# savage-hacker14/audio-to-sheet-music

Hardware: AMD Instinct MI355X
Metric: 6s-segments/sec (each separated into 4 stems; encode once, decode 4x) (higher is better)
Workload: dtype bf16; 1 GPU; BASELINE configs[2]: B=64 x 6 s segments x 4 prompts per GPU; global_batch=64, seq_len=264600, prompts=4, parallelism=segment-sharded dp1, launch=hipGraph replay of one athd_forward_prompts per step (1 graph(s) per rank), pipelines=1, decode_items=256

## Files before the change

audio-to-sheet-music_amd/csrc/fdec_lr.hip:

```cpp
#include <algorithm>
#include <cstdlib>

#include "common.h"
#include "kernels.h"
#include "prof.h"

namespace athd {

namespace {

typedef float f2 __attribute__((ext_vector_type(2)));
typedef __bf16 bf2_t __attribute__((ext_vector_type(2)));

ATHD_DEV f2 splat(float v) { return (f2){v, v}; }
ATHD_DEV f2 pfma(f2 a, f2 b, f2 c) { return __builtin_elementwise_fma(a, b, c); }

template <typename T>
ATHD_DEV f2 ld2(const T* p) {
    if constexpr (sizeof(T) == 2) {
        const uint32_t q = *reinterpret_cast<const uint32_t*>(p);
        return (f2){__uint_as_float(q << 16), __uint_as_float(q & 0xFFFF0000u)};
    } else {
        return *reinterpret_cast<const f2*>(p);
    }
}

template <bool FAST>
ATHD_DEV f2 gelu2(f2 x) {
    if constexpr (!FAST) {
        return (f2){gelu_erf(x.x), gelu_erf(x.y)};
    } else {
        return (f2){gelu_fast(x.x), gelu_fast(x.y)};
    }
}

ATHD_DEV f2 gelu2_pk(f2 x) {
    const f2 u = x * pfma(splat(0.044715f * 1.5957691216057308f), x * x, splat(1.5957691216057308f));
    const f2 t = u * splat(-1.4426950408889634f);
    const f2 den = (f2){__builtin_amdgcn_exp2f(t.x), __builtin_amdgcn_exp2f(t.y)} + splat(1.0f);
    return x * (f2){__builtin_amdgcn_rcpf(den.x), __builtin_amdgcn_rcpf(den.y)};
}

template <typename ZT, int NT>
ATHD_DEV void load_rows(const ZT* base, int64_t rowpitch, int Co, int i0, int i1, float scale, f2 (&r0)[NT],
                        f2 (&dr)[NT]);

template <int NT>
ATHD_DEV constexpr int tap_of(int t) { return NT == 8 ? t : (t == 0 ? 0 : t == 1 ? 3 : t == 2 ? 4 : 7); }

template <typename ZT, int NT>
ATHD_DEV void load_rows(const ZT* base, int64_t rowpitch, int Co, int i0, int i1, float scale, f2 (&r0)[NT],
                        f2 (&dr)[NT]) {
    f2 a[NT], b[NT];
#pragma unroll
    for (int t = 0; t < NT; ++t) a[t] = ld2(base + (int64_t)i0 * rowpitch + tap_of<NT>(t) * Co);
#pragma unroll
    for (int t = 0; t < NT; ++t) b[t] = ld2(base + (int64_t)i1 * rowpitch + tap_of<NT>(t) * Co);
#pragma unroll
    for (int t = 0; t < NT; ++t) {
        r0[t] = a[t] * splat(scale);
        dr[t] = (b[t] - a[t]) * splat(scale);
    }
}

struct LrThread {
    int item, seg, w, c;
    bool active;
};

ATHD_DEV LrThread lr_thread(const LowRankDesc& d) {
    LrThread t;
    const int cg = d.Co / 2;
    const int q = blockIdx.x * 256 + threadIdx.x;
    t.active = q < d.W * cg;
    t.w = t.active ? q / cg : 0;
    t.c = t.active ? (q % cg) * 2 : 0;
    t.item = blockIdx.y;
    t.seg = t.item / d.P;
    return t;
}

}

typedef uint32_t u32x4_t __attribute__((ext_vector_type(4)));
typedef __attribute__((address_space(4))) const u32x4_t c_u32x4;
ATHD_DEV LrStep lr_step(const LrStep* steps, int v) {
    static_assert(sizeof(LrStep) == 32, "LrStep layout");
    const c_u32x4* p = (const c_u32x4*)steps + 2 * __builtin_amdgcn_readfirstlane(v);
    const u32x4_t a = p[0], b = p[1];
    LrStep e;
    e.lz = __uint_as_float(a.x);
    e.lk = __uint_as_float(a.y);
    e.lj = __uint_as_float(a.z);
    e.zk = a.w;
    e.jj = b.x;
    e.flags = b.y;
    return e;
}

__global__ __launch_bounds__(256) void fdec_lr_steps_kernel(LrStep* steps, int Hd, int Hs, int Hk, int H_skip) {
    for (int v = threadIdx.x; v <= Hd; v += blockDim.x) {
        LrStep e = {};
        int z0 = -1, z1 = -1, k0 = -1, k1 = -1, j0 = -1, j1 = -1, pz0 = -2, pz1 = -2, pk0 = -2, pk1 = -2, pj0 = -2,
            pj1 = -2;
        if (v < Hd) {
            const LinIdx a = lin_index(v, Hs, Hd), k = lin_index(v, Hk, Hd);
            z0 = a.i0; z1 = a.i1; k0 = k.i0; k1 = k.i1;
            e.lz = a.l1;
            e.lk = k.l1;
        }
        if (v >= 1) {
            const LinIdx j = lin_index(v - 1, H_skip, Hd);
            j0 = j.i0; j1 = j.i1;
            e.lj = j.l1;
            if (v - 1 < Hd) {
                const LinIdx pa = lin_index(v - 1, Hs, Hd), pk = lin_index(v - 1, Hk, Hd);
                pz0 = pa.i0; pz1 = pa.i1; pk0 = pk.i0; pk1 = pk.i1;
            }
            if (v >= 2) {
                const LinIdx pj = lin_index(v - 2, H_skip, Hd);
// ... 55 lines not shown
                    const f2 y1 = T[3] + prev[3];
                    a1 += y0 + y1;
                    a2 = pfma(y0, y0, pfma(y1, y1, a2));
                }
#pragma unroll
                for (int t = 0; t < 4; ++t) prev[t] = T[4 + t];
            }
            s1 += (double)a1.x + (double)a1.y;
            s2 += (double)a2.x + (double)a2.y;
        }
    }
    s1 = wave_sum_d(s1);
    s2 = wave_sum_d(s2);
    __shared__ double sh[2][4];
    const int wv = threadIdx.x >> 6;
    if ((threadIdx.x & 63) == 0) { sh[0][wv] = s1; sh[1][wv] = s2; }
    __syncthreads();
    if (threadIdx.x == 0) {
        atomicAdd(&d.stats[2 * th.item], sh[0][0] + sh[0][1] + sh[0][2] + sh[0][3]);
        atomicAdd(&d.stats[2 * th.item + 1], sh[1][0] + sh[1][1] + sh[1][2] + sh[1][3]);
    }
}

ATHD_DEV f2 bf2u(uint32_t q) { return (f2){__uint_as_float(q << 16), __uint_as_float(q & 0xFFFF0000u)}; }

__global__ __launch_bounds__(256) void fdec_lr_stats3_kernel(const LowRankDesc d) {
    const LrThread th = lr_thread(d);
    const int N8 = 8 * d.Co;
    const int64_t rp = (int64_t)d.W * N8;
    const bf16_t* zb = (const bf16_t*)d.Z + (int64_t)th.item * d.Hs * rp + (int64_t)th.w * N8 + th.c;
    const bf16_t* sb = (const bf16_t*)d.Zs + (int64_t)th.seg * d.Hk * rp + (int64_t)th.w * N8 + th.c;
    const f2 bias = ld2(d.bias + th.c);
    f2 zhi[8], zdr[8], shi[8], sdr[8], base[8];
    uint32_t zpf[8], spf[8];
    double s1 = 0.0, s2 = 0.0;
    auto ldrow = [&](const bf16_t* p, int row, uint32_t (&r)[8]) {
#pragma unroll
        for (int t = 0; t < 8; ++t) r[t] = *reinterpret_cast<const uint32_t*>(p + (int64_t)row * rp + t * d.Co);
    };
    if (th.active) {
        const LrStep s0 = lr_step(d.steps, 0);
        int zr = (s0.zk >> 8) & 0xFF, kr = s0.zk >> 24;
        {
            uint32_t za[8], ka[8];
            ldrow(zb, s0.zk & 0xFF, za);
            ldrow(zb, zr, zpf);
            ldrow(sb, (s0.zk >> 16) & 0xFF, ka);
            ldrow(sb, kr, spf);
// ... 68 lines not shown
            a1 = f2{};
            a2 = f2{};
        }
        a1 += pv[0] + pv[1];
        a2 = pfma(pv[0], pv[0], pfma(pv[1], pv[1], a2));
        s1 += (double)a1.x + (double)a1.y;
        s2 += (double)a2.x + (double)a2.y;
    }
    s1 = wave_sum_d(s1);
    s2 = wave_sum_d(s2);
    __shared__ double sh[2][4];
    const int wv = threadIdx.x >> 6;
    if ((threadIdx.x & 63) == 0) { sh[0][wv] = s1; sh[1][wv] = s2; }
    __syncthreads();
    if (threadIdx.x == 0) {
        atomicAdd(&d.stats[2 * th.item], sh[0][0] + sh[0][1] + sh[0][2] + sh[0][3]);
        atomicAdd(&d.stats[2 * th.item + 1], sh[1][0] + sh[1][1] + sh[1][2] + sh[1][3]);
    }
}

__global__ __launch_bounds__(256) void fdec_lr_merge3_kernel(const LowRankDesc d) {
    const LrThread th = lr_thread(d);
    if (!th.active) return;
    constexpr int NT = 4;
    const int N8 = 8 * d.Co, NZ = d.z_taps * d.Co;
    const int64_t rp = (int64_t)d.W * N8, rpz = (int64_t)d.W * NZ;
    const bool z4 = d.z_taps == 4;
    const bf16_t* zb = (const bf16_t*)d.Z + (int64_t)th.item * d.Hs * rpz + (int64_t)th.w * NZ +
                       (z4 ? (th.c >> 4) * 64 + (th.c & 15) : th.c);
    const bf16_t* sb = (const bf16_t*)d.Zs + (int64_t)th.seg * d.Hk * rp + (int64_t)th.w * N8 + th.c;
    float mean, rstd;
    gn_params(d.stats, th.item, 4LL * d.Hd * d.W * d.Co, mean, rstd);
    const f2 bias = ld2(d.bias + th.c);
    const f2 gsc = ld2(d.gn_w + th.c) * splat(rstd);
    const f2 gb = ld2(d.gn_b + th.c) - splat(mean) * gsc;
    const int64_t kp = (int64_t)d.W * d.C_skip;
    const bf16_t* kbp = (const bf16_t*)d.skip + (int64_t)th.seg * d.H_skip * kp + (int64_t)th.w * d.C_skip + th.c;
    bf2_t* op = (bf2_t*)((bf16_t*)d.out + (int64_t)th.item * d.Hd * d.W * d.Co + (int64_t)th.w * d.Co + th.c);
    const int64_t ostep = (int64_t)d.W * d.Co / 2;

    auto ldrow = [&](const bf16_t* p, int row, uint32_t (&r)[NT], bool compact) {
#pragma unroll
        for (int t = 0; t < NT; ++t)
            r[t] = *reinterpret_cast<const uint32_t*>(p + (int64_t)row * (compact ? rpz : rp) +
                                                      (compact ? t * 16 : tap_of<NT>(t) * d.Co));
    };
    f2 zhi[NT], zdr[NT], shi[NT], sdr[NT], base[NT];
    uint32_t zpf[NT], spf[NT];
    const LrStep s0 = lr_step(d.steps, 0);
    int zr = (s0.zk >> 8) & 0xFF, kr = s0.zk >> 24;
    {
        uint32_t za[NT], ka[NT];
        ldrow(zb, s0.zk & 0xFF, za, z4);
        ldrow(zb, zr, zpf, z4);
        ldrow(sb, (s0.zk >> 16) & 0xFF, ka, false);
        ldrow(sb, kr, spf, false);
#pragma unroll
        for (int t = 0; t < NT; ++t) {
            const f2 a = bf2u(za[t]), b = bf2u(zpf[t]);
            const f2 ka2 = bf2u(ka[t]) * splat(0.1f), kb2 = bf2u(spf[t]) * splat(0.1f);
            zhi[t] = b;
            zdr[t] = b - a;
            shi[t] = kb2;
            sdr[t] = kb2 - ka2;
            base[t] = a + ka2 + ((t == 1 || t == 2) ? bias : f2{});
        }
    }
    ldrow(zb, min(zr + 1, d.Hs - 1), zpf, z4);
    ldrow(sb, min(kr + 1, d.Hk - 1), spf, false);
    const LrStep s1e = lr_step(d.steps, 1);
    int jr = (int)(s1e.jj >> 16);
    f2 khi, kdr;
    uint32_t jpf;
    {
        const f2 a = bf2u(*reinterpret_cast<const uint32_t*>(kbp + (int64_t)(s1e.jj & 0xFFFF) * kp)) * splat(0.1f);
        khi = bf2u(*reinterpret_cast<const uint32_t*>(kbp + (int64_t)jr * kp)) * splat(0.1f);
        kdr = khi - a;
    }
    jpf = *reinterpret_cast<const uint32_t*>(kbp + (int64_t)min(jr + 1, d.H_skip - 1) * kp);
    f2 kbase = khi - kdr;

    auto tstep = [&](const LrStep& st, f2 (&T)[NT]) {
        if (st.flags & 1u) {
#pragma unroll
            for (int t = 0; t < NT; ++t) {
                const f2 nb = bf2u(zpf[t]);
                base[t] += zdr[t];
                zdr[t] = nb - zhi[t];
                zhi[t] = nb;
            }
            zr = min(zr + 1, d.Hs - 1);
            ldrow(zb, min(zr + 1, d.Hs - 1), zpf, z4);
        }
        if (st.flags & 2u) {
#pragma unroll
            for (int t = 0; t < NT; ++t) {
                const f2 nb = bf2u(spf[t]) * splat(0.1f);
                base[t] += sdr[t];
                sdr[t] = nb - shi[t];
                shi[t] = nb;
            }
            kr = min(kr + 1, d.Hk - 1);
            ldrow(sb, min(kr + 1, d.Hk - 1), spf, false);
        }
#pragma unroll
        for (int t = 0; t < NT; ++t) T[t] = pfma(splat(st.lz), zdr[t], pfma(splat(st.lk), sdr[t], base[t]));
    };
    auto emit = [&](const LrStep& st, f2 y1, f2 y2, int dd) {
        if (dd >= 1 && (st.flags & 4u)) {
            const f2 nb = bf2u(jpf) * splat(0.1f);
            kbase += kdr;
            kdr = nb - khi;
            khi = nb;
            jr = min(jr + 1, d.H_skip - 1);
            jpf = *reinterpret_cast<const uint32_t*>(kbp + (int64_t)min(jr + 1, d.H_skip - 1) * kp);
        }
        const f2 gs = gelu_fast_wsum_pk(splat(0.5f), pfma(y1, gsc, gb), splat(0.5f), pfma(y2, gsc, gb));
        const f2 o = gs + pfma(splat(st.lj), kdr, kbase);
        op[(int64_t)dd * ostep] = __builtin_convertvector(o, bf2_t);
    };
    f2 cur3, cur4, cur7, prev7 = {};
    {
        f2 T[NT];
#pragma unroll
        for (int t = 0; t < NT; ++t) T[t] = pfma(splat(s0.lz), zdr[t], pfma(splat(s0.lk), sdr[t], base[t]));
        cur3 = T[1];
        cur4 = T[2];
        cur7 = T[3];
    }
    LrStep nx = s1e;
    for (int v = 1; v < d.Hd; ++v) {
        const LrStep st = nx;
        nx = lr_step(d.steps, v + 1);
        f2 T[NT];
        tstep(st, T);
        emit(st, cur3 + prev7, cur4 + T[0], v - 1);
        prev7 = cur7;
        cur3 = T[1];
        cur4 = T[2];
        cur7 = T[3];
    }
    emit(nx, cur3 + prev7, cur4, d.Hd - 1);
}

template <typename ZT, bool FAST>
__global__ __launch_bounds__(256) void fdec_lr_merge2_kernel(const LowRankDesc d) {
    const LrThread th = lr_thread(d);
    if (!th.active) return;
    const int N8 = 8 * d.Co;
    const int64_t rp = (int64_t)d.W * N8;
    const ZT* zb = (const ZT*)d.Z + (int64_t)th.item * d.Hs * rp + (int64_t)th.w * N8 + th.c;
    const ZT* sb = (const ZT*)d.Zs + (int64_t)th.seg * d.Hk * rp + (int64_t)th.w * N8 + th.c;
    float mean, rstd;
    gn_params(d.stats, th.item, 4LL * d.Hd * d.W * d.Co, mean, rstd);
    const f2 bias = ld2(d.bias + th.c);
    const f2 gsc = ld2(d.gn_w + th.c) * splat(rstd);
    const f2 gb = ld2(d.gn_b + th.c);
    const int64_t kp = (int64_t)d.W * d.C_skip;
    const int64_t kb = (int64_t)th.seg * d.H_skip * kp + (int64_t)th.w * d.C_skip + th.c;
    f2 ka = {}, kd = {};
    const int64_t ob = (int64_t)th.item * d.Hd * d.W * d.Co + (int64_t)th.w * d.Co + th.c;
    const int64_t op = (int64_t)d.W * d.Co;

    f2 zr0[4], zdr[4], sr0[4], sdr[4];
    f2 base[4];
// ... 126 lines not shown
```

audio-to-sheet-music_amd/csrc/forward.h:

```cpp
#pragma once
#include <hip/hip_runtime.h>

#include <algorithm>
#include <cstdio>
#include <cstdlib>
#include <string>
#include <vector>

#include "../../include/athd.h"
#include "attn.h"
#include "ctx.h"
#include "gemm.h"
#include "kernels.h"
#include "prof.h"

namespace athd_fwd {

struct Dims {
    int64_t B = 0, T = 0;
    int P = 1, Tspec = 0;
    int F[5] = {2048, 512, 128, 32, 8};
    int64_t L[5] = {0, 0, 0, 0, 0};
    int64_t Nf = 0, Nt = 0, Nmax = 0;
    int64_t Bc = 0, chunks = 0;
// ... 19 lines not shown
    float *avec, *tc0, *tc2;
    float *Yb, *x_cond, *xt_cond;
    void* Hm;
    float* Ybt;
    void* Hmt;
    float *G, *D, *FO;
    float* FO2 = nullptr;
    float* ola_part;
    LrStep* lrsteps;
    float* gram;
    double* gramq;
    void *S, *Z, *Zs;
    float* skw[2] = {nullptr, nullptr};
};

inline void* eoff(void* p, int64_t n, int ea) { return (char*)p + n * ea; }

struct Switches {
    static bool env(const char* name, bool dflt) {
        const char* e = std::getenv(name);
        return dflt ? !(e && *e == '0') : (e && *e && *e != '0');
    }
    bool serial = env("ATHD_SERIAL", false), sk = env("ATHD_SK", true), rowln = env("ATHD_ROWLN", true),
         fdec1_fused = env("ATHD_FDEC1_FUSED", true), fenc_row = env("ATHD_FENC_ROW", true);
};

struct Status {
    int err = 0;
    std::string what;
    void check(int rc, const char* w) { if (rc != 0 && err == 0) { err = rc; what = w; } }
};

enum Branch { MAIN = 0, TIME = 1 };
struct StreamPlan {
    hipStream_t main, time;
    hipEvent_t ev_f, ev_t;
    bool serial;
    Status* st;

    StreamPlan(athd_ctx* c, hipStream_t caller, bool serial_, Status* st_)
        : main(caller), time(serial_ ? caller : c->s_time), ev_f(c->ev_f), ev_t(c->ev_t), serial(serial_), st(st_) {
        if (!c->s_time || !c->ev_f || !c->ev_t) st->check((int)hipErrorInvalidResourceHandle, "second stream");
    }
    void record(hipEvent_t ev, hipStream_t s) { st->check((int)hipEventRecord(ev, s), "event record"); }
    void wait(hipStream_t s, hipEvent_t ev) { st->check((int)hipStreamWaitEvent(s, ev, 0), "event wait"); }
    void fork() { record(ev_f, main); wait(time, ev_f); }
    void join() { record(ev_t, time); wait(main, ev_t); }
// ... 74 lines not shown
```

audio-to-sheet-music_amd/csrc/forward_dec.cpp:

```cpp
#include "forward.h"

namespace athd_fwd {
namespace {

void conv_t(Run& r, const DecW& w, const void* A, int a_bf16, int nb, int H_in, int W, void* out, int out_bf16,
            double* st, int keep, const char* stage) {
    KStage kst(stage);
    if (w.ct4w && a_bf16 && out_bf16 && convt4_supported(w.cin, w.cout, nb, H_in, W)) {
        ConvT4Desc q;
        q.x = (const uint16_t*)A; q.w = w.ct4w; q.bias = w.ct4b; q.out = (uint16_t*)out; q.stats = st;
        q.nb = nb; q.H = H_in; q.W = W; q.keep = keep < 0 ? 0 : 1;
        r.check(convt4_launch(q, r.s), "convt4");
        return;
    }
    auto residues = [&](const GemmW& gw, int ntaps, int in_off) {
        GemmDesc g = conv_h(gw, A, a_bf16, nb, H_in, W, w.cin, ntaps, 1, in_off, 1, H_in);
        out_to(g, out, out_bf16, w.cout, (keep < 0 ? 4 : 2) * H_in);
        g.o_stride = keep < 0 ? 4 : 2;
        g.stats = st; g.col_split = w.cout;
        return g;
    };
    if (w.quad.w) {
        GemmDesc g = residues(w.quad, 3, -1);
        if (w.cin % 32 == 0) g.k_blk = w.cin;
// ... 58 lines not shown
    else gn_gelu_launch(b.G, NI, 32 * Ts * 192, 192, st, c->fdec[0].gnw, c->fdec[0].gnb, r.s, false);
    KStage kst1("fdec1");
    const DecW& w1 = c->fdec[1];
    GemmDesc gz = conv1(w1.taps, r.actbf ? b.S : (const void*)b.G, ab, NI, 32, Ts, w1.cin);
    out_to(gz, b.Z, ab, w1.taps.N, 32);
    LowRankDesc lr;
    lr.steps = b.lrsteps;
    lr.Z = b.Z; lr.Zs = b.Zs; lr.z_bf16 = ab; lr.Hs = 32; lr.Hk = 8; lr.Hd = (int)Ts; lr.W = (int)Ts;
    lr.Co = w1.cout; lr.P = P; lr.NI = NI; lr.bias = w1.bias; lr.stats = r.stats(NI);
    lr.gn_w = w1.gnw; lr.gn_b = w1.gnb; lr.fast_gelu = ab;
    lr.skip = sv[2]; lr.skip_bf16 = ab; lr.H_skip = 32; lr.C_skip = 192;
    lr.out = b.D; lr.out_bf16 = ab;
    lr.S = gz.A; lr.Wt = w1.taps.w; lr.w_ld = w1.taps.Kp; lr.Ci = w1.cin;
    const bool gram = r.sw.fdec1_fused && b.gram && fdec1_gram_supported(lr);
    if (gram) { lr.z_taps = 4; lr.z4 = b.Z; }
    else r.gemm(gz, "fdec1.z");
    GemmDesc gs = conv1(w1.taps, sv[3], ab, Bc, 8, Ts, w1.cin);
    gs.a_ld = 384;
    out_to(gs, b.Zs, ab, w1.taps.N, 8);
    r.gemm(gs, "fdec1.zs");
    r.check(fdec_lr_steps_launch(b.lrsteps, (int)Ts, 32, 8, 32, r.s), "fdec_lr_steps");
    if (gram) r.check(fdec1_gram_launch(lr, b.gram, b.gramq, r.s), "fdec1_gram");
    else r.check(fdec_lr_stats_launch(lr, r.s), "fdec_lr_stats");
    r.check(fdec_lr_merge_launch(lr, r.s), "fdec_lr_merge");
    const DecW& w = c->fdec[2];
    double* sti = r.stats(NI);
    conv_t(r, w, b.D, ab, NI, (int)Ts, (int)Ts, b.G, ab, sti, 1, "fdec2");
    KStage kst3("fdec3");
    DecLastDesc dl;
    dl.g = b.G; dl.g_bf16 = ab; dl.stats = sti; dl.gn_count = 4 * Ts * Ts * w.cout; dl.gn_w = w.gnw; dl.gn_b = w.gnb;
    dl.fast_gelu = ab; dl.skip2 = sv[1]; dl.skip2_bf16 = ab; dl.H_skip2 = 128; dl.C_skip2 = 96;
    dl.H = (int)Ts; dl.W = (int)Ts;
    last_level(dl, c->flast, eoff(b.sk4, s0 * 512 * Ts * 4, ea), 512);
    dl.out = FO;
    r.check(fdec_tail_launch(dl, r.s), "fdec_tail");
}

float* Chunk::time_decoder() const {
    const void* svt[4] = {eoff(b.saved_t[0], s0 * d.L[1] * 48, b.ea), eoff(b.saved_t[1], s0 * d.L[2] * 96, b.ea),
                          eoff(b.saved_t[2], s0 * d.L[3] * 192, b.ea), eoff(b.saved_t[3], s0 * d.L[4] * 384, b.ea)};
    const void* const sk4t = eoff(b.sk4t, s0 * d.L[1] * 4, b.ea);
    const void* A = b.xt_cond;
    int64_t Lin = d.Nt;
    static const char* const kT[3] = {"tdec0", "tdec1", "tdec2"};
    for (int i = 0; i < 3; ++i) {
        const DecW& w = c->tdec[i];
        double* st = r.stats(NI);
        conv_t(r, w, A, ab, NI, (int)Lin, 1, b.Gt, ab, st, -1, kT[i]);
        KStage kst(kT[i]);
        const int64_t target = d.L[3 - i];
// ... 61 lines not shown
```

audio-to-sheet-music_amd/csrc/kernels.h:

```cpp
#pragma once
#include <hip/hip_runtime.h>
#include <stdint.h>

#include "../../include/athd.h"
#include "gemm.h"

namespace athd {

struct PadPlan {
    int64_t L;
    int64_t left;
    int64_t ext_left;
    int64_t Lx;
};
inline PadPlan stft_pad_plan(int64_t T, int64_t Tspec) {
    const int64_t pl = 1536, pr = 1536 + Tspec * 1024 - T, maxpad = pl > pr ? pl : pr;
    const int64_t extra = T <= maxpad ? maxpad - T + 1 : 0, epr = pr < extra ? pr : extra, epl = extra - epr;
    PadPlan pp;
    pp.L = T; pp.left = pl - epl; pp.ext_left = epl; pp.Lx = T + epl + epr;
    return pp;
}

void tconv0_launch(const float* wav, int nb, int64_t T, int64_t Lo, const float* w, const float* bias,
                   const float* tnorm, void* out, int out_bf16, hipStream_t s);
// ... 105 lines not shown
    float* out = nullptr;
    const void* g = nullptr; int g_bf16 = 0; int Hg = 0;
    const double* stats = nullptr; int64_t gn_count = 0; const float* gn_w = nullptr; const float* gn_b = nullptr;
    int fast_gelu = 0;
    const void* skip2 = nullptr; int skip2_bf16 = 0; int H_skip2 = 0; int C_skip2 = 0;
};
int fdec_last_launch(const DecLastDesc& d, hipStream_t s);
int tdec_last_launch(const DecLastDesc& d, hipStream_t s);
int fdec_tail_launch(const DecLastDesc& d, hipStream_t s);
bool tdec_tail_supported(const DecLastDesc& d);
int tdec_tail_launch(const DecLastDesc& d, hipStream_t s);
struct ConvT4Desc {
    const uint16_t* x = nullptr;
    const uint16_t* w = nullptr;
    const float* bias = nullptr;
    uint16_t* out = nullptr;
    double* stats = nullptr;
    int nb = 0, H = 0, W = 1, keep = 0;
    uint32_t M = 0;
    FastDivU fd_w, fd_h, fd_hw;
};
bool convt4_supported(int cin, int cout, int64_t nb, int64_t H, int64_t W);
int convt4_launch(const ConvT4Desc& d, hipStream_t s);
inline bool dconv_narrow(int C) { return C == 48 || C == 96; }
inline bool dconv_bf16(int mode) { return mode == 1; }
struct DconvPlan {
    bool ok;
    bool valu;
    bool conv3_mfma;
    enum Norm { MOM, BF16, F32 } norm;
    bool apply_mfma;
    bool rewrite;
};
DconvPlan dconv_plan(int mode, int C, int64_t nb, int64_t L, bool rewrite_fusable);
struct DconvDesc {
    void* x = nullptr; int x_bf16 = 0;
    float* h = nullptr;
    uint16_t* hb = nullptr;
    double *st_h = nullptr, *st_y = nullptr;
    int64_t M = 0, L = 0; int C = 0, dil = 1;
    const float *w3f = nullptr, *w1f = nullptr;
    bool fast = false;
    const uint16_t *w3 = nullptr, *w1 = nullptr;
    int w3_kp = 0, w1_kp = 0;
    const float *b3 = nullptr, *g1w = nullptr, *g1b = nullptr, *scale = nullptr;
    const float *b1 = nullptr, *g2w = nullptr, *g2b = nullptr;
// ... 105 lines not shown
```

audio-to-sheet-music_amd/csrc/ktest.cpp:

```cpp
#include <hip/hip_runtime.h>
#include <stdint.h>
#include <string.h>

#include "attn.h"
#include "ctx.h"
#include "forward.h"
#include "gemm.h"
#include "kernels.h"
#include "pack.h"
#include "text_tower.h"

namespace athd {
int dec_merge_run();
int dec_merge_maxp();
int dec_last_const(int which);
int fdec1_gram_wb();
int fdec1_gram_blocks();
}

using namespace athd;

extern "C" {

struct KtGemm {
// ... 257 lines not shown
    d.C_skip = (int)k->C_skip; d.P = (int)k->P; d.out = k->out; d.out_bf16 = (int)k->out_bf16; d.H_out = (int)k->H_out;
    d.W = (int)k->W; d.NI = (int)k->NI; d.proj_w = (const float*)k->proj_w; d.proj_b = (const float*)k->proj_b;
    d.fast_gelu = (int)k->fast_gelu;
    return dec_merge_launch(d, (hipStream_t)stream);
}
static LowRankDesc to_lr(const KtLowRank* k) {
    LowRankDesc d;
    d.steps = (const LrStep*)k->steps; d.Z = k->Z; d.Zs = k->Zs; d.z_bf16 = (int)k->z_bf16; d.z_taps = (int)k->z_taps;
    d.Hs = (int)k->Hs; d.Hk = (int)k->Hk; d.Hd = (int)k->Hd; d.W = (int)k->W; d.Co = (int)k->Co; d.P = (int)k->P;
    d.NI = (int)k->NI; d.bias = (const float*)k->bias; d.stats = (double*)k->stats; d.gn_w = (const float*)k->gn_w;
    d.gn_b = (const float*)k->gn_b; d.fast_gelu = (int)k->fast_gelu; d.skip = k->skip; d.skip_bf16 = (int)k->skip_bf16;
    d.H_skip = (int)k->H_skip; d.C_skip = (int)k->C_skip; d.out = k->out; d.out_bf16 = (int)k->out_bf16;
    d.S = k->S; d.Wt = k->Wt; d.w_ld = (int)k->w_ld; d.Ci = (int)k->Ci; d.z4 = k->z4;
    return d;
}
int kt_fdec_lr_stats(const KtLowRank* k, void* stream) { return fdec_lr_stats_launch(to_lr(k), (hipStream_t)stream); }
int kt_fdec_lr_merge(const KtLowRank* k, void* stream) { return fdec_lr_merge_launch(to_lr(k), (hipStream_t)stream); }
int kt_fdec1_gram(const KtLowRank* k, void* stream) {
    return fdec1_gram_launch(to_lr(k), (float*)k->gram, (double*)k->gq, (hipStream_t)stream);
}
int kt_fdec1_gram_supported(const KtLowRank* k) { return fdec1_gram_supported(to_lr(k)); }
int kt_fdec_lr_steps(void* steps, int64_t Hd, int64_t Hs, int64_t Hk, int64_t H_skip, void* stream) {
    return fdec_lr_steps_launch((LrStep*)steps, (int)Hd, (int)Hs, (int)Hk, (int)H_skip, (hipStream_t)stream);
}
int64_t kt_fdec1_gram_floats(int64_t NI, int64_t W) { return fdec1_gram_floats(NI, (int)W); }
int64_t kt_fdec1_gram_q_doubles() { return fdec1_gram_q_doubles(); }
static DecLastDesc to_dl(const KtDecLast* k) {
    DecLastDesc d;
    d.in = k->in; d.in_bf16 = (int)k->in_bf16; d.NI = (int)k->NI; d.P = (int)k->P; d.H = (int)k->H; d.W = (int)k->W;
    d.T = k->T; d.fold = (const float*)k->fold; d.skip = k->skip; d.skip_bf16 = (int)k->skip_bf16;
    d.H_skip = (int)k->H_skip; d.C_skip = (int)k->C_skip; d.out = (float*)k->out; d.g = k->g; d.g_bf16 = (int)k->g_bf16;
    d.Hg = (int)k->Hg; d.stats = (const double*)k->stats; d.gn_count = k->gn_count; d.gn_w = (const float*)k->gn_w;
    d.gn_b = (const float*)k->gn_b; d.fast_gelu = (int)k->fast_gelu; d.skip2 = k->skip2; d.skip2_bf16 = (int)k->skip2_bf16;
    d.H_skip2 = (int)k->H_skip2; d.C_skip2 = (int)k->C_skip2;
    return d;
}
int kt_fdec_last(const KtDecLast* k, void* stream) { return fdec_last_launch(to_dl(k), (hipStream_t)stream); }
int kt_tdec_last(const KtDecLast* k, void* stream) { return tdec_last_launch(to_dl(k), (hipStream_t)stream); }
int kt_fdec_tail(const KtDecLast* k, void* stream) { return fdec_tail_launch(to_dl(k), (hipStream_t)stream); }
int kt_tdec_tail(const KtDecLast* k, void* stream) { return tdec_tail_launch(to_dl(k), (hipStream_t)stream); }
int kt_tdec_tail_supported(const KtDecLast* k) { return tdec_tail_supported(to_dl(k)); }
int64_t kt_fl_dc() { return dec_last_const(0); }
int64_t kt_ft_dc() { return dec_last_const(1); }
int64_t kt_tl_in() { return dec_last_const(2); }
int64_t kt_tt_rows() { return dec_last_const(3); }
int64_t kt_dm_run() { return dec_merge_run(); }
// ... 176 lines not shown
```

Baseline: 1853 segments/s.

## Fuse low-rank merge with fdec2 transposed conv via LDS ring producer/consumer kernel

```diff
diff --git a/audio-to-sheet-music_amd/csrc/fdec12.hip b/audio-to-sheet-music_amd/csrc/fdec12.hip
--- /dev/null
+++ b/audio-to-sheet-music_amd/csrc/fdec12.hip
@@ -0,0 +1,198 @@
+#include <algorithm>
+
+#include "common.h"
+#include "fdec_lr_merge3.h"
+#include "gemm.h"
+#include "gemm_tile.h"
+#include "kernels.h"
+#include "prof.h"
+
+namespace athd {
+
+namespace {
+
+constexpr int CT_CI = 96, CT_CO = 48;
+constexpr int CT_KP = 2 * CT_CI;
+constexpr int CT_WROW = CT_KP * 2;
+constexpr int F12_R = FDEC12_R, F12_SLOTS = 2 * F12_R;
+constexpr int F12_ROWB = FDEC12_WB * CT_CI * 2;
+constexpr int F12_NP = 12, F12_NC = 4;
+constexpr int F12_OSB = FDEC12_WB * CT_CO * 2;
+static_assert((F12_SLOTS & (F12_SLOTS - 1)) == 0, "ring slots: a power of two");
+static_assert(F12_NP * 64 == FDEC12_WB * (CT_CI / 2), "one producer thread per (column, channel pair)");
+
+ATHD_DEV int ring_chunk(int w, int ch) { return (ch & 12) | ((ch ^ (0 - (w >> 2))) & 3); }
+
+}
+
+__global__ __launch_bounds__(1024) void fdec12_kernel(const LowRankDesc d, const ConvT4Desc q, const Fdec12Plan plan) {
+    __shared__ __attribute__((aligned(16))) char wl[4 * CT_CO * CT_WROW];
+    __shared__ __attribute__((aligned(16))) char ring[F12_SLOTS * F12_ROWB];
+    __shared__ __attribute__((aligned(16))) char ostg[2][F12_OSB];
+    __shared__ double ssum[2][F12_NC][2];
+    if (fdec12_task(plan, (int)blockIdx.x, 0) < 0) return;
+    for (int c = threadIdx.x; c < 4 * CT_CO * 24; c += 1024) {
+        const int n = c / 24, ch = c - 24 * (c / 24);
+        const uint4 v = reinterpret_cast<const uint4*>(q.w)[c];
+        *reinterpret_cast<uint4*>(wl + n * CT_WROW + ((ch ^ (n & 7)) * 16)) = v;
+    }
+    __syncthreads();
+
+    const int lane = threadIdx.x & 63;
+    const int wave = __builtin_amdgcn_readfirstlane(threadIdx.x >> 6);
+    const int Hd = d.Hd, W = d.W;
+    const int phases = plan.phases;
+
+    if (wave < F12_NP) {
+        const int wl_ = threadIdx.x / (CT_CI / 2), c = (threadIdx.x % (CT_CI / 2)) * 2;
+        char* const slot0 = ring + wl_ * (CT_CI * 2) + ring_chunk(wl_, c >> 3) * 16 + (c & 7) * 2;
+        for (int k = 0;; ++k) {
+            const int t = fdec12_task(plan, (int)blockIdx.x, k);
+            if (t < 0) break;
+            const int wblk = t / d.NI, item = t - wblk * d.NI;
+            const int w = min(FDEC12_WB * wblk + wl_, W - 1);
+            lr_merge3_rows(d, item, item / d.P, w, c, [&](int dd, bf2_t v) {
+                *reinterpret_cast<bf2_t*>(slot0 + (dd & (F12_SLOTS - 1)) * F12_ROWB) = v;
+                if (((dd + 1) & (F12_R - 1)) == 0) __syncthreads();
+            });
+            for (int ph = Hd / F12_R; ph < phases; ++ph) __syncthreads();
+        }
+        return;
+    }
+
+    const int rho = wave - F12_NP;
+    const int fr = lane & 15, g = lane >> 4;
+    const bool stored = rho == 1 || rho == 2;
+    float4 b4[3];
+#pragma unroll
+    for (int jj = 0; jj < 3; ++jj) b4[jj] = *reinterpret_cast<const float4*>(q.bias + 16 * jj + 4 * g);
+    const int f7 = fr & 7;
+    const uint32_t wrho = (uint32_t)((96 * (rho >> 1) + 16 * 3 * (rho & 1)) * CT_WROW);
+    uint32_t wbe = wrho + (uint32_t)(fr * CT_WROW + (4 * (f7 >> 2) + (g ^ (f7 & 3))) * 16);
+    uint32_t wbo = wrho + (uint32_t)(fr * CT_WROW + (4 * (1 - (f7 >> 2)) + (g ^ (f7 & 3))) * 16);
+    auto wfrag = [&](int jj, int s) -> bf16v8 {
+        const uint32_t a = ((s & 1) ? wbo : wbe) + (uint32_t)(16 * jj * CT_WROW + 128 * (s >> 1));
+        return *reinterpret_cast<const bf16v8*>(wl + a);
+    };
+    const uint32_t roff = (uint32_t)(fr * (CT_CI * 2) + ring_chunk(fr, g) * 16);
+    const f32x4_t z4 = {0.f, 0.f, 0.f, 0.f};
+    f32x4_t acc[3];
+    bf16v8 wf[3][3];
+    auto wload = [&](int gi) {
+        __builtin_amdgcn_sched_barrier(0);
+#pragma unroll
+        for (int jj = 0; jj < 3; ++jj) wf[gi % 3][jj] = wfrag(jj, gi);
+        __builtin_amdgcn_sched_barrier(0);
+    };
+    auto mma = [&](int h, const bf16v8 (&F)[3]) {
+#pragma unroll
+        for (int s = 0; s < 3; ++s) {
+#pragma unroll
+            for (int jj = 0; jj < 3; ++jj)
+                acc[jj] = __builtin_amdgcn_mfma_f32_16x16x32_bf16(wf[s][jj], F[s], (h == 0 && s == 0) ? z4 : acc[jj], 0, 0, 0);
+            wload((3 * h + s + 3) % 6);
+        }
+    };
+    wload(0);
+    wload(1);
+    wload(2);
+    const bf16v8 zf = __builtin_bit_cast(bf16v8, make_uint4(0u, 0u, 0u, 0u));
+    char* const stage = ostg[stored ? rho - 1 : 0];
+
+    for (int k = 0;; ++k) {
+        const int t = fdec12_task(plan, (int)blockIdx.x, k);
+        if (t < 0) break;
+        const int wblk = t / d.NI, item = t - wblk * d.NI;
+        const bool cok = FDEC12_WB * wblk + fr < W;
+        char* const oitem = reinterpret_cast<char*>(q.out) + (int64_t)item * Hd * 2 * W * (CT_CO * 2);
+        const int64_t orowB = (int64_t)W * (CT_CO * 2);
+        const int ocol0 = FDEC12_WB * wblk * (CT_CO * 2);
+        const int ovalid = min(FDEC12_WB, W - FDEC12_WB * wblk) * (CT_CO * 2);
+        double r1 = 0.0, r2 = 0.0;
+        bf16v8 lo[3] = {zf, zf, zf}, up[3];
+        __syncthreads();
+        for (int ph = 1; ph < phases; ++ph) {
+            const int rend = min(ph * F12_R, Hd + 1);
+#pragma unroll 1
+            for (int r = (ph - 1) * F12_R; r < rend; ++r) {
+                if (r < Hd) {
+                    const char* const rp = ring + (r & (F12_SLOTS - 1)) * F12_ROWB + roff;
+#pragma unroll
+                    for (int s3 = 0; s3 < 3; ++s3) up[s3] = *reinterpret_cast<const bf16v8*>(rp + 64 * s3);
+                } else {
+#pragma unroll
+                    for (int s3 = 0; s3 < 3; ++s3) up[s3] = zf;
+                }
+                const int u = rho < 2 ? r : r - 1;
+                if (u >= 0 && u < Hd) {
+                    mma(0, lo);
+                    mma(1, up);
+                    float p1 = 0.f, p2 = 0.f;
+#pragma unroll
+                    for (int jj = 0; jj < 3; ++jj) {
+                        const float4 bb = b4[jj];
+                        const float v0 = acc[jj][0] + bb.x, v1 = acc[jj][1] + bb.y;
+                        const float v2 = acc[jj][2] + bb.z, v3 = acc[jj][3] + bb.w;
+                        p1 += (v0 + v1) + (v2 + v3);
+                        p2 += (v0 * v0 + v1 * v1) + (v2 * v2 + v3 * v3);
+                        if (stored)
+                            *reinterpret_cast<uint2*>(stage + fr * (CT_CO * 2) + 32 * jj + 8 * g) =
+                                make_uint2(pack2bf(v0, v1), pack2bf(v2, v3));
+                    }
+                    r1 += (double)(cok ? p1 : 0.f);
+                    r2 += (double)(cok ? p2 : 0.f);
+                    if (stored) {
+                        asm volatile("s_waitcnt lgkmcnt(0)" ::: "memory");
+                        __builtin_amdgcn_wave_barrier();
+                        char* const orow = oitem + (int64_t)(2 * u + rho - 1) * orowB + ocol0;
+#pragma unroll
+                        for (int kk = 0; kk < (F12_OSB / 16 + 63) / 64; ++kk) {
+                            const int wb = (lane + 64 * kk) * 16;
+                            if (wb < ovalid) *reinterpret_cast<uint4*>(orow + wb) = *reinterpret_cast<const uint4*>(stage + wb);
+                        }
+                    }
+                }
+#pragma unroll
+                for (int s3 = 0; s3 < 3; ++s3) lo[s3] = up[s3];
+            }
+            if (ph == phases - 1) {
+                const double t1 = wave_sum_d(r1), t2 = wave_sum_d(r2);
+                if (lane == 0) { ssum[k & 1][rho][0] = t1; ssum[k & 1][rho][1] = t2; }
+            }
+            __syncthreads();
+        }
+        if (rho == 0 && lane == 0) {
+            const double (&s)[F12_NC][2] = ssum[k & 1];
+            atomicAdd(&q.stats[2 * item], (s[0][0] + s[1][0]) + (s[2][0] + s[3][0]));
+            atomicAdd(&q.stats[2 * item + 1], (s[0][1] + s[1][1]) + (s[2][1] + s[3][1]));
+        }
+    }
+}
+
+bool fdec12_supported(const LowRankDesc& d, const ConvT4Desc& q) {
+    return d.steps && d.Z && d.Zs && d.bias && d.stats && d.gn_w && d.gn_b && d.skip && q.w && q.bias && q.out && q.stats &&
+           d.z_bf16 && d.skip_bf16 && d.fast_gelu && d.z_taps == 4 && d.Co == CT_CI && d.C_skip >= d.Co && d.C_skip % 2 == 0 &&
+           d.Hs > 0 && d.Hs <= 256 && d.Hk > 0 && d.Hk <= 256 && d.H_skip > 0 && d.Hd > d.Hs && d.Hd > d.Hk && d.Hd > d.H_skip &&
+           d.Hd < 65536 && d.W >= FDEC12_WB && d.P > 0 && d.NI > 0 && d.NI % d.P == 0 && q.keep == 1 && q.nb == d.NI &&
+           q.H == d.Hd && q.W == d.W && (int64_t)d.NI * ((d.W + FDEC12_WB - 1) / FDEC12_WB) < (1LL << 31) &&
+           convt4_supported(CT_CI, CT_CO, q.nb, q.H, q.W);
+}
+
+int fdec12_launch(const LowRankDesc& d, const ConvT4Desc& q, hipStream_t s) {
+    if (!fdec12_supported(d, q)) return -1;
+    const Fdec12Plan plan = fdec12_plan(d.NI, d.Hd, d.W, device_cus());
+    KScope ks(s);
+    if (ks.on()) {
+        const double M = (double)d.NI * d.Hd * d.W;
+        const double flops = 2.0 * M * (4 * CT_CO) * CT_KP;
+        const double segs = (double)(d.NI / d.P);
+        const double bytes = 2.0 * 4.0 * d.Co * d.W * ((double)d.NI * d.Hs + segs * d.Hk) +
+                             segs * std::min<double>(d.H_skip, 2.0 * d.Hd) * d.W * d.Co * 2.0 + M * 2 * CT_CO * 2 +
+                             4.0 * CT_CO * CT_KP * 2;
+        ks.begin("fdec12_kernel", flops, bytes);
+    }
+    hipLaunchKernelGGL(fdec12_kernel, dim3((unsigned)plan.blocks), dim3(1024), 0, s, d, q, plan);
+    return (int)hipGetLastError();
+}
+
+}
diff --git a/audio-to-sheet-music_amd/csrc/fdec_lr.hip b/audio-to-sheet-music_amd/csrc/fdec_lr.hip
--- a/audio-to-sheet-music_amd/csrc/fdec_lr.hip
+++ b/audio-to-sheet-music_amd/csrc/fdec_lr.hip
@@ -2,18 +2,13 @@
 #include <cstdlib>
 
 #include "common.h"
+#include "fdec_lr_merge3.h"
 #include "kernels.h"
 #include "prof.h"
 
 namespace athd {
 
 namespace {
-
-typedef float f2 __attribute__((ext_vector_type(2)));
-typedef __bf16 bf2_t __attribute__((ext_vector_type(2)));
-
-ATHD_DEV f2 splat(float v) { return (f2){v, v}; }
-ATHD_DEV f2 pfma(f2 a, f2 b, f2 c) { return __builtin_elementwise_fma(a, b, c); }
 
 template <typename T>
 ATHD_DEV f2 ld2(const T* p) {
@@ -44,9 +39,6 @@
 template <typename ZT, int NT>
 ATHD_DEV void load_rows(const ZT* base, int64_t rowpitch, int Co, int i0, int i1, float scale, f2 (&r0)[NT],
                         f2 (&dr)[NT]);
-
-template <int NT>
-ATHD_DEV constexpr int tap_of(int t) { return NT == 8 ? t : (t == 0 ? 0 : t == 1 ? 3 : t == 2 ? 4 : 7); }
 
 template <typename ZT, int NT>
 ATHD_DEV void load_rows(const ZT* base, int64_t rowpitch, int Co, int i0, int i1, float scale, f2 (&r0)[NT],
@@ -80,22 +72,6 @@
     return t;
 }
 
-}
-
-typedef uint32_t u32x4_t __attribute__((ext_vector_type(4)));
-typedef __attribute__((address_space(4))) const u32x4_t c_u32x4;
-ATHD_DEV LrStep lr_step(const LrStep* steps, int v) {
-    static_assert(sizeof(LrStep) == 32, "LrStep layout");
-    const c_u32x4* p = (const c_u32x4*)steps + 2 * __builtin_amdgcn_readfirstlane(v);
-    const u32x4_t a = p[0], b = p[1];
-    LrStep e;
-    e.lz = __uint_as_float(a.x);
-    e.lk = __uint_as_float(a.y);
-    e.lj = __uint_as_float(a.z);
-    e.zk = a.w;
-    e.jj = b.x;
-    e.flags = b.y;
-    return e;
 }
 
 __global__ __launch_bounds__(256) void fdec_lr_steps_kernel(LrStep* steps, int Hd, int Hs, int Hk, int H_skip) {
@@ -197,8 +173,6 @@
     }
 }
 
-ATHD_DEV f2 bf2u(uint32_t q) { return (f2){__uint_as_float(q << 16), __uint_as_float(q & 0xFFFF0000u)}; }
-
 __global__ __launch_bounds__(256) void fdec_lr_stats3_kernel(const LowRankDesc d) {
     const LrThread th = lr_thread(d);
     const int N8 = 8 * d.Co;
@@ -313,125 +287,9 @@
 __global__ __launch_bounds__(256) void fdec_lr_merge3_kernel(const LowRankDesc d) {
     const LrThread th = lr_thread(d);
     if (!th.active) return;
-    constexpr int NT = 4;
-    const int N8 = 8 * d.Co, NZ = d.z_taps * d.Co;
-    const int64_t rp = (int64_t)d.W * N8, rpz = (int64_t)d.W * NZ;
-    const bool z4 = d.z_taps == 4;
-    const bf16_t* zb = (const bf16_t*)d.Z + (int64_t)th.item * d.Hs * rpz + (int64_t)th.w * NZ +
-                       (z4 ? (th.c >> 4) * 64 + (th.c & 15) : th.c);
-    const bf16_t* sb = (const bf16_t*)d.Zs + (int64_t)th.seg * d.Hk * rp + (int64_t)th.w * N8 + th.c;
-    float mean, rstd;
-    gn_params(d.stats, th.item, 4LL * d.Hd * d.W * d.Co, mean, rstd);
-    const f2 bias = ld2(d.bias + th.c);
-    const f2 gsc = ld2(d.gn_w + th.c) * splat(rstd);
-    const f2 gb = ld2(d.gn_b + th.c) - splat(mean) * gsc;
-    const int64_t kp = (int64_t)d.W * d.C_skip;
-    const bf16_t* kbp = (const bf16_t*)d.skip + (int64_t)th.seg * d.H_skip * kp + (int64_t)th.w * d.C_skip + th.c;
     bf2_t* op = (bf2_t*)((bf16_t*)d.out + (int64_t)th.item * d.Hd * d.W * d.Co + (int64_t)th.w * d.Co + th.c);
     const int64_t ostep = (int64_t)d.W * d.Co / 2;
-
-    auto ldrow = [&](const bf16_t* p, int row, uint32_t (&r)[NT], bool compact) {
-#pragma unroll
-        for (int t = 0; t < NT; ++t)
-            r[t] = *reinterpret_cast<const uint32_t*>(p + (int64_t)row * (compact ? rpz : rp) +
-                                                      (compact ? t * 16 : tap_of<NT>(t) * d.Co));
-    };
-    f2 zhi[NT], zdr[NT], shi[NT], sdr[NT], base[NT];
-    uint32_t zpf[NT], spf[NT];
-    const LrStep s0 = lr_step(d.steps, 0);
-    int zr = (s0.zk >> 8) & 0xFF, kr = s0.zk >> 24;
-    {
-        uint32_t za[NT], ka[NT];
-        ldrow(zb, s0.zk & 0xFF, za, z4);
-        ldrow(zb, zr, zpf, z4);
-        ldrow(sb, (s0.zk >> 16) & 0xFF, ka, false);
-        ldrow(sb, kr, spf, false);
-#pragma unroll
-        for (int t = 0; t < NT; ++t) {
-            const f2 a = bf2u(za[t]), b = bf2u(zpf[t]);
-            const f2 ka2 = bf2u(ka[t]) * splat(0.1f), kb2 = bf2u(spf[t]) * splat(0.1f);
-            zhi[t] = b;
-            zdr[t] = b - a;
-            shi[t] = kb2;
-            sdr[t] = kb2 - ka2;
-            base[t] = a + ka2 + ((t == 1 || t == 2) ? bias : f2{});
-        }
-    }
-    ldrow(zb, min(zr + 1, d.Hs - 1), zpf, z4);
-    ldrow(sb, min(kr + 1, d.Hk - 1), spf, false);
-    const LrStep s1e = lr_step(d.steps, 1);
-    int jr = (int)(s1e.jj >> 16);
-    f2 khi, kdr;
-    uint32_t jpf;
-    {
-        const f2 a = bf2u(*reinterpret_cast<const uint32_t*>(kbp + (int64_t)(s1e.jj & 0xFFFF) * kp)) * splat(0.1f);
-        khi = bf2u(*reinterpret_cast<const uint32_t*>(kbp + (int64_t)jr * kp)) * splat(0.1f);
-        kdr = khi - a;
-    }
-    jpf = *reinterpret_cast<const uint32_t*>(kbp + (int64_t)min(jr + 1, d.H_skip - 1) * kp);
-    f2 kbase = khi - kdr;
-
-    auto tstep = [&](const LrStep& st, f2 (&T)[NT]) {
-        if (st.flags & 1u) {
-#pragma unroll
-            for (int t = 0; t < NT; ++t) {
-                const f2 nb = bf2u(zpf[t]);
-                base[t] += zdr[t];
-                zdr[t] = nb - zhi[t];
-                zhi[t] = nb;
-            }
-            zr = min(zr + 1, d.Hs - 1);
-            ldrow(zb, min(zr + 1, d.Hs - 1), zpf, z4);
-        }
-        if (st.flags & 2u) {
-#pragma unroll
-            for (int t = 0; t < NT; ++t) {
-                const f2 nb = bf2u(spf[t]) * splat(0.1f);
-                base[t] += sdr[t];
-                sdr[t] = nb - shi[t];
-                shi[t] = nb;
-            }
-            kr = min(kr + 1, d.Hk - 1);
-            ldrow(sb, min(kr + 1, d.Hk - 1), spf, false);
-        }
-#pragma unroll
-        for (int t = 0; t < NT; ++t) T[t] = pfma(splat(st.lz), zdr[t], pfma(splat(st.lk), sdr[t], base[t]));
-    };
-    auto emit = [&](const LrStep& st, f2 y1, f2 y2, int dd) {
-        if (dd >= 1 && (st.flags & 4u)) {
-            const f2 nb = bf2u(jpf) * splat(0.1f);
-            kbase += kdr;
-            kdr = nb - khi;
-            khi = nb;
-            jr = min(jr + 1, d.H_skip - 1);
-            jpf = *reinterpret_cast<const uint32_t*>(kbp + (int64_t)min(jr + 1, d.H_skip - 1) * kp);
-        }
-        const f2 gs = gelu_fast_wsum_pk(splat(0.5f), pfma(y1, gsc, gb), splat(0.5f), pfma(y2, gsc, gb));
-        const f2 o = gs + pfma(splat(st.lj), kdr, kbase);
-        op[(int64_t)dd * ostep] = __builtin_convertvector(o, bf2_t);
-    };
-    f2 cur3, cur4, cur7, prev7 = {};
-    {
-        f2 T[NT];
-#pragma unroll
-        for (int t = 0; t < NT; ++t) T[t] = pfma(splat(s0.lz), zdr[t], pfma(splat(s0.lk), sdr[t], base[t]));
-        cur3 = T[1];
-        cur4 = T[2];
-        cur7 = T[3];
-    }
-    LrStep nx = s1e;
-    for (int v = 1; v < d.Hd; ++v) {
-        const LrStep st = nx;
-        nx = lr_step(d.steps, v + 1);
-        f2 T[NT];
-        tstep(st, T);
-        emit(st, cur3 + prev7, cur4 + T[0], v - 1);
-        prev7 = cur7;
-        cur3 = T[1];
-        cur4 = T[2];
-        cur7 = T[3];
-    }
-    emit(nx, cur3 + prev7, cur4, d.Hd - 1);
+    lr_merge3_rows(d, th.item, th.seg, th.w, th.c, [&](int dd, bf2_t v) { op[(int64_t)dd * ostep] = v; });
 }
 
 template <typename ZT, bool FAST>
diff --git a/audio-to-sheet-music_amd/csrc/fdec_lr_merge3.h b/audio-to-sheet-music_amd/csrc/fdec_lr_merge3.h
--- /dev/null
+++ b/audio-to-sheet-music_amd/csrc/fdec_lr_merge3.h
@@ -0,0 +1,156 @@
+#pragma once
+#include "common.h"
+#include "kernels.h"
+
+namespace athd {
+namespace {
+
+typedef float f2 __attribute__((ext_vector_type(2)));
+typedef __bf16 bf2_t __attribute__((ext_vector_type(2)));
+
+ATHD_DEV f2 splat(float v) { return (f2){v, v}; }
+ATHD_DEV f2 pfma(f2 a, f2 b, f2 c) { return __builtin_elementwise_fma(a, b, c); }
+ATHD_DEV f2 bf2u(uint32_t q) { return (f2){__uint_as_float(q << 16), __uint_as_float(q & 0xFFFF0000u)}; }
+
+template <int NT>
+ATHD_DEV constexpr int tap_of(int t) { return NT == 8 ? t : (t == 0 ? 0 : t == 1 ? 3 : t == 2 ? 4 : 7); }
+
+typedef uint32_t u32x4_t __attribute__((ext_vector_type(4)));
+typedef __attribute__((address_space(4))) const u32x4_t c_u32x4;
+ATHD_DEV LrStep lr_step(const LrStep* steps, int v) {
+    static_assert(sizeof(LrStep) == 32, "LrStep layout");
+    const c_u32x4* p = (const c_u32x4*)steps + 2 * __builtin_amdgcn_readfirstlane(v);
+    const u32x4_t a = p[0], b = p[1];
+    LrStep e;
+    e.lz = __uint_as_float(a.x);
+    e.lk = __uint_as_float(a.y);
+    e.lj = __uint_as_float(a.z);
+    e.zk = a.w;
+    e.jj = b.x;
+    e.flags = b.y;
+    return e;
+}
+
+template <typename Sink>
+ATHD_DEV void lr_merge3_rows(const LowRankDesc& d, int item, int seg, int w, int c, Sink&& sink) {
+    constexpr int NT = 4;
+    const int N8 = 8 * d.Co, NZ = d.z_taps * d.Co;
+    const int64_t rp = (int64_t)d.W * N8, rpz = (int64_t)d.W * NZ;
+    const bool z4 = d.z_taps == 4;
+    const bf16_t* zb = (const bf16_t*)d.Z + (int64_t)item * d.Hs * rpz + (int64_t)w * NZ +
+                       (z4 ? (c >> 4) * 64 + (c & 15) : c);
+    const bf16_t* sb = (const bf16_t*)d.Zs + (int64_t)seg * d.Hk * rp + (int64_t)w * N8 + c;
+    float mean, rstd;
+    gn_params(d.stats, item, 4LL * d.Hd * d.W * d.Co, mean, rstd);
+    const f2 bias = *reinterpret_cast<const f2*>(d.bias + c);
+    const f2 gsc = *reinterpret_cast<const f2*>(d.gn_w + c) * splat(rstd);
+    const f2 gb = *reinterpret_cast<const f2*>(d.gn_b + c) - splat(mean) * gsc;
+    const int64_t kp = (int64_t)d.W * d.C_skip;
+    const bf16_t* kbp = (const bf16_t*)d.skip + (int64_t)seg * d.H_skip * kp + (int64_t)w * d.C_skip + c;
+
+    auto ldrow = [&](const bf16_t* p, int row, uint32_t (&r)[NT], bool compact) {
+#pragma unroll
+        for (int t = 0; t < NT; ++t)
+            r[t] = *reinterpret_cast<const uint32_t*>(p + (int64_t)row * (compact ? rpz : rp) +
+                                                      (compact ? t * 16 : tap_of<NT>(t) * d.Co));
+    };
+    f2 zhi[NT], zdr[NT], shi[NT], sdr[NT], base[NT];
+    uint32_t zpf[NT], spf[NT];
+    const LrStep s0 = lr_step(d.steps, 0);
+    int zr = (s0.zk >> 8) & 0xFF, kr = s0.zk >> 24;
+    {
+        uint32_t za[NT], ka[NT];
+        ldrow(zb, s0.zk & 0xFF, za, z4);
+        ldrow(zb, zr, zpf, z4);
+        ldrow(sb, (s0.zk >> 16) & 0xFF, ka, false);
+        ldrow(sb, kr, spf, false);
+#pragma unroll
+        for (int t = 0; t < NT; ++t) {
+            const f2 a = bf2u(za[t]), b = bf2u(zpf[t]);
+            const f2 ka2 = bf2u(ka[t]) * splat(0.1f), kb2 = bf2u(spf[t]) * splat(0.1f);
+            zhi[t] = b;
+            zdr[t] = b - a;
+            shi[t] = kb2;
+            sdr[t] = kb2 - ka2;
+            base[t] = a + ka2 + ((t == 1 || t == 2) ? bias : f2{});
+        }
+    }
+    ldrow(zb, min(zr + 1, d.Hs - 1), zpf, z4);
+    ldrow(sb, min(kr + 1, d.Hk - 1), spf, false);
+    const LrStep s1e = lr_step(d.steps, 1);
+    int jr = (int)(s1e.jj >> 16);
+    f2 khi, kdr;
+    uint32_t jpf;
+    {
+        const f2 a = bf2u(*reinterpret_cast<const uint32_t*>(kbp + (int64_t)(s1e.jj & 0xFFFF) * kp)) * splat(0.1f);
+        khi = bf2u(*reinterpret_cast<const uint32_t*>(kbp + (int64_t)jr * kp)) * splat(0.1f);
+        kdr = khi - a;
+    }
+    jpf = *reinterpret_cast<const uint32_t*>(kbp + (int64_t)min(jr + 1, d.H_skip - 1) * kp);
+    f2 kbase = khi - kdr;
+
+    auto tstep = [&](const LrStep& st, f2 (&T)[NT]) {
+        if (st.flags & 1u) {
+#pragma unroll
+            for (int t = 0; t < NT; ++t) {
+                const f2 nb = bf2u(zpf[t]);
+                base[t] += zdr[t];
+                zdr[t] = nb - zhi[t];
+                zhi[t] = nb;
+            }
+            zr = min(zr + 1, d.Hs - 1);
+            ldrow(zb, min(zr + 1, d.Hs - 1), zpf, z4);
+        }
+        if (st.flags & 2u) {
+#pragma unroll
+            for (int t = 0; t < NT; ++t) {
+                const f2 nb = bf2u(spf[t]) * splat(0.1f);
+                base[t] += sdr[t];
+                sdr[t] = nb - shi[t];
+                shi[t] = nb;
+            }
+            kr = min(kr + 1, d.Hk - 1);
+            ldrow(sb, min(kr + 1, d.Hk - 1), spf, false);
+        }
+#pragma unroll
+        for (int t = 0; t < NT; ++t) T[t] = pfma(splat(st.lz), zdr[t], pfma(splat(st.lk), sdr[t], base[t]));
+    };
+    auto emit = [&](const LrStep& st, f2 y1, f2 y2, int dd) {
+        if (dd >= 1 && (st.flags & 4u)) {
+            const f2 nb = bf2u(jpf) * splat(0.1f);
+            kbase += kdr;
+            kdr = nb - khi;
+            khi = nb;
+            jr = min(jr + 1, d.H_skip - 1);
+            jpf = *reinterpret_cast<const uint32_t*>(kbp + (int64_t)min(jr + 1, d.H_skip - 1) * kp);
+        }
+        const f2 gs = gelu_fast_wsum_pk(splat(0.5f), pfma(y1, gsc, gb), splat(0.5f), pfma(y2, gsc, gb));
+        const f2 o = gs + pfma(splat(st.lj), kdr, kbase);
+        sink(dd, __builtin_convertvector(o, bf2_t));
+    };
+    f2 cur3, cur4, cur7, prev7 = {};
+    {
+        f2 T[NT];
+#pragma unroll
+        for (int t = 0; t < NT; ++t) T[t] = pfma(splat(s0.lz), zdr[t], pfma(splat(s0.lk), sdr[t], base[t]));
+        cur3 = T[1];
+        cur4 = T[2];
+        cur7 = T[3];
+    }
+    LrStep nx = s1e;
+    for (int v = 1; v < d.Hd; ++v) {
+        const LrStep st = nx;
+        nx = lr_step(d.steps, v + 1);
+        f2 T[NT];
+        tstep(st, T);
+        emit(st, cur3 + prev7, cur4 + T[0], v - 1);
+        prev7 = cur7;
+        cur3 = T[1];
+        cur4 = T[2];
+        cur7 = T[3];
+    }
+    emit(nx, cur3 + prev7, cur4, d.Hd - 1);
+}
+
+}
+}
diff --git a/audio-to-sheet-music_amd/csrc/forward.h b/audio-to-sheet-music_amd/csrc/forward.h
--- a/audio-to-sheet-music_amd/csrc/forward.h
+++ b/audio-to-sheet-music_amd/csrc/forward.h
@@ -65,7 +65,8 @@
         return dflt ? !(e && *e == '0') : (e && *e && *e != '0');
     }
     bool serial = env("ATHD_SERIAL", false), sk = env("ATHD_SK", true), rowln = env("ATHD_ROWLN", true),
-         fdec1_fused = env("ATHD_FDEC1_FUSED", true), fenc_row = env("ATHD_FENC_ROW", true);
+         fdec1_fused = env("ATHD_FDEC1_FUSED", true), fdec12_fused = env("ATHD_FDEC12_FUSED", true),
+         fenc_row = env("ATHD_FENC_ROW", true);
 };
 
 struct Status {
diff --git a/audio-to-sheet-music_amd/csrc/forward_dec.cpp b/audio-to-sheet-music_amd/csrc/forward_dec.cpp
--- a/audio-to-sheet-music_amd/csrc/forward_dec.cpp
+++ b/audio-to-sheet-music_amd/csrc/forward_dec.cpp
@@ -104,10 +104,18 @@
     r.check(fdec_lr_steps_launch(b.lrsteps, (int)Ts, 32, 8, 32, r.s), "fdec_lr_steps");
     if (gram) r.check(fdec1_gram_launch(lr, b.gram, b.gramq, r.s), "fdec1_gram");
     else r.check(fdec_lr_stats_launch(lr, r.s), "fdec_lr_stats");
-    r.check(fdec_lr_merge_launch(lr, r.s), "fdec_lr_merge");
     const DecW& w = c->fdec[2];
     double* sti = r.stats(NI);
-    conv_t(r, w, b.D, ab, NI, (int)Ts, (int)Ts, b.G, ab, sti, 1, "fdec2");
+    ConvT4Desc q2;
+    q2.x = (const uint16_t*)b.D; q2.w = w.ct4w; q2.bias = w.ct4b; q2.out = (uint16_t*)b.G; q2.stats = sti;
+    q2.nb = NI; q2.H = (int)Ts; q2.W = (int)Ts; q2.keep = 1;
+    if (r.sw.fdec12_fused && ab && w.cin == lr.Co && fdec12_supported(lr, q2)) {
+        KStage kst2("fdec2");
+        r.check(fdec12_launch(lr, q2, r.s), "fdec12");
+    } else {
+        r.check(fdec_lr_merge_launch(lr, r.s), "fdec_lr_merge");
+        conv_t(r, w, b.D, ab, NI, (int)Ts, (int)Ts, b.G, ab, sti, 1, "fdec2");
+    }
     KStage kst3("fdec3");
     DecLastDesc dl;
     dl.g = b.G; dl.g_bf16 = ab; dl.stats = sti; dl.gn_count = 4 * Ts * Ts * w.cout; dl.gn_w = w.gnw; dl.gn_b = w.gnb;
diff --git a/audio-to-sheet-music_amd/csrc/kernels.h b/audio-to-sheet-music_amd/csrc/kernels.h
--- a/audio-to-sheet-music_amd/csrc/kernels.h
+++ b/audio-to-sheet-music_amd/csrc/kernels.h
@@ -151,6 +151,24 @@
 };
 bool convt4_supported(int cin, int cout, int64_t nb, int64_t H, int64_t W);
 int convt4_launch(const ConvT4Desc& d, hipStream_t s);
+constexpr int FDEC12_WB = 16, FDEC12_R = 8;
+struct Fdec12Plan { int nwb, tasks, blocks, phases; };
+inline Fdec12Plan fdec12_plan(int NI, int Hd, int W, int cus) {
+    Fdec12Plan p;
+    p.nwb = (W + FDEC12_WB - 1) / FDEC12_WB;
+    p.tasks = NI * p.nwb;
+    p.blocks = ((cus < p.tasks ? cus : p.tasks) + 7) / 8 * 8;
+    p.phases = Hd / FDEC12_R + 2;
+    return p;
+}
+__host__ __device__ inline int fdec12_task(const Fdec12Plan& p, int block, int k) {
+    const int xcd = block & 7;
+    const int i0 = (int)((int64_t)p.tasks * xcd / 8), i1 = (int)((int64_t)p.tasks * (xcd + 1) / 8);
+    const int64_t t = (int64_t)i0 + (block >> 3) + (int64_t)k * (p.blocks >> 3);
+    return t < i1 ? (int)t : -1;
+}
+bool fdec12_supported(const LowRankDesc& lr, const ConvT4Desc& ct);
+int fdec12_launch(const LowRankDesc& lr, const ConvT4Desc& ct, hipStream_t s);
 inline bool dconv_narrow(int C) { return C == 48 || C == 96; }
 inline bool dconv_bf16(int mode) { return mode == 1; }
 struct DconvPlan {
diff --git a/audio-to-sheet-music_amd/csrc/ktest.cpp b/audio-to-sheet-music_amd/csrc/ktest.cpp
--- a/audio-to-sheet-music_amd/csrc/ktest.cpp
+++ b/audio-to-sheet-music_amd/csrc/ktest.cpp
@@ -303,6 +303,23 @@
 int kt_fdec1_gram_supported(const KtLowRank* k) { return fdec1_gram_supported(to_lr(k)); }
 int kt_fdec_lr_steps(void* steps, int64_t Hd, int64_t Hs, int64_t Hk, int64_t H_skip, void* stream) {
     return fdec_lr_steps_launch((LrStep*)steps, (int)Hd, (int)Hs, (int)Hk, (int)H_skip, (hipStream_t)stream);
+}
+static ConvT4Desc to_ct4(const KtConvT4* k) {
+    ConvT4Desc c;
+    c.x = (const uint16_t*)k->x; c.w = (const uint16_t*)k->w; c.bias = (const float*)k->bias; c.out = (uint16_t*)k->out;
+    c.stats = (double*)k->stats; c.nb = (int)k->nb; c.H = (int)k->H; c.W = (int)k->W; c.keep = (int)k->keep;
+    return c;
+}
+int kt_fdec12(const KtLowRank* k, const KtConvT4* c, void* stream) {
+    return fdec12_launch(to_lr(k), to_ct4(c), (hipStream_t)stream);
+}
+int kt_fdec12_supported(const KtLowRank* k, const KtConvT4* c) { return fdec12_supported(to_lr(k), to_ct4(c)); }
+void kt_fdec12_plan(int64_t NI, int64_t Hd, int64_t W, int64_t cus, int64_t* out) {
+    const Fdec12Plan p = fdec12_plan((int)NI, (int)Hd, (int)W, (int)cus);
+    out[0] = p.nwb; out[1] = p.tasks; out[2] = p.blocks; out[3] = p.phases; out[4] = FDEC12_R;
+}
+int64_t kt_fdec12_task(int64_t NI, int64_t Hd, int64_t W, int64_t cus, int64_t block, int64_t k) {
+    return fdec12_task(fdec12_plan((int)NI, (int)Hd, (int)W, (int)cus), (int)block, (int)k);
 }
 int64_t kt_fdec1_gram_floats(int64_t NI, int64_t W) { return fdec1_gram_floats(NI, (int)W); }
 int64_t kt_fdec1_gram_q_doubles() { return fdec1_gram_q_doubles(); }
```

Result: faster. 1877 segments/s, median of 6 (+1.3%).
